# rohitsinghlab/SAME

Hardware: AMD Instinct MI355X
Metric: cell-pairs/sec on 100k×100k cost build + edge-cross sweep; % HBM roofline (higher is better)
Workload: dtype f64

## Files before the change

same_amd/csrc/window_finish.hip:

```cpp
#include "assign.h"
#include "refine.h"

namespace {

using namespace devmath;
using namespace win;
using scan::Pair;

struct FilterArgs {
    const double *xy;
    const int32_t *raw;
    int64_t Tr, n;
    const int32_t *type_id;
    uint8_t *cls;
    double *perim;
    uint8_t *has_kept, *any_valid;
    unsigned long long *best_p;
    unsigned *best_t, *first_v;
    unsigned long long *st_keep, *st_own, *counters;
    int32_t *klist, *nlist, *out;
};

__global__ __launch_bounds__(256) void filter_classify_kernel(Batch<FilterArgs> b, double radius, int angle_enabled, double cos_thr, int near_enabled,
                                                               double tol) {
    const FilterArgs &w = b.w[blockIdx.y];
    if ((int64_t)blockIdx.x * blockDim.x >= w.Tr) return;
    const int64_t t = (int64_t)blockIdx.x * blockDim.x + threadIdx.x;
    const int32_t *__restrict__ tris = w.raw, *__restrict__ type_id = w.type_id;
    bool near = false;
    if (t < w.Tr) {
        const int32_t a = tris[3 * t], bb = tris[3 * t + 1], d = tris[3 * t + 2];
        const TriClass r = classify_triangle(ld2(w.xy, a), ld2(w.xy, bb), ld2(w.xy, d), radius, angle_enabled, cos_thr,
                                             type_id && type_id[a] == type_id[bb] && type_id[bb] == type_id[d]);
        w.cls[t] = r.cls;
        w.perim[t] = r.perim;
        near = near_enabled && r.cls != 1 && fabs(r.maxcos - cos_thr) <= tol;
        if (r.cls == 0 || r.cls == 3) {
            w.any_valid[a] = 1; w.any_valid[bb] = 1; w.any_valid[d] = 1;
            if (r.cls == 0) { w.has_kept[a] = 1; w.has_kept[bb] = 1; w.has_kept[d] = 1; }
        }
        if (w.best_p && r.cls == 3) {
            const unsigned long long key = ~(unsigned long long)__double_as_longlong(r.perim);
            atomicMax(&w.best_p[a], key); atomicMax(&w.best_p[bb], key); atomicMax(&w.best_p[d], key);
        }
    }
    const unsigned long long nb = __ballot(near);
    if ((threadIdx.x & 63) == 0 && nb) atomicAdd(&w.counters[FC_NEAR], (unsigned long long)__builtin_popcountll(nb));
}
__global__ __launch_bounds__(scan::NT) void filter_keep_kernel(Batch<FilterArgs> b) {
    __shared__ scan::Shared sh;
    const FilterArgs &w = b.w[blockIdx.y];
    const int nb = (int)scan::blocks_for(w.Tr);
    if ((int)blockIdx.x >= nb || w.Tr == 0) return;
    const int64_t Tr = w.Tr;
    const uint8_t *__restrict__ cls = w.cls;
    auto val = [&](int64_t t) { return Pair{t < Tr && cls[t] == 0 ? 1u : 0u, 0u}; };
    Pair through;
    const Pair off = scan::exclusive(w.st_keep, (int)blockIdx.x, val, sh, &through);
    const int64_t t = (int64_t)blockIdx.x * scan::NT + threadIdx.x;
    if (t < Tr) {
        const uint8_t c = cls[t];
        if (c == 0) w.klist[off.a] = (int32_t)t;
        if (w.best_p && c == 3) {
            const unsigned long long key = ~(unsigned long long)__double_as_longlong(w.perim[t]);
            for (int q = 0; q < 3; ++q) {
                const int32_t v = w.raw[3 * t + q];
                if (w.best_p[v] == key) atomicMax(&w.best_t[v], ~(unsigned)t);
            }
        }
    }
    if ((int)blockIdx.x == nb - 1 && threadIdx.x == 0) w.counters[FC_KEEP] = through.a;
}
__device__ __forceinline__ bool asks(const uint8_t *has_kept, const uint8_t *any_valid, const unsigned *best_t, int64_t v) {
    return !has_kept[v] && any_valid[v] && best_t[v] != 0u;
}
__global__ __launch_bounds__(256) void filter_first_node_kernel(Batch<FilterArgs> b) {
    const FilterArgs &w = b.w[blockIdx.y];
    const int64_t v = (int64_t)blockIdx.x * blockDim.x + threadIdx.x;
    if (v >= w.n || !asks(w.has_kept, w.any_valid, w.best_t, v)) return;
    atomicMax(&w.first_v[~w.best_t[v]], ~(unsigned)v);
}
__global__ __launch_bounds__(scan::NT) void filter_owner_kernel(Batch<FilterArgs> b) {
    __shared__ scan::Shared sh;
    const FilterArgs &w = b.w[blockIdx.y];
    const int nb = (int)scan::blocks_for(w.n);
    if ((int)blockIdx.x >= nb || w.n == 0) return;
    const int64_t n = w.n;
    auto own = [&](int64_t v) { return v < n && asks(w.has_kept, w.any_valid, w.best_t, v) && w.first_v[~w.best_t[v]] == ~(unsigned)v; };
    auto val = [&](int64_t v) { return Pair{own(v) ? 1u : 0u, 0u}; };
    Pair through;
    const Pair off = scan::exclusive(w.st_own, (int)blockIdx.x, val, sh, &through);
    const int64_t v = (int64_t)blockIdx.x * scan::NT + threadIdx.x;
    if (own(v)) w.nlist[off.a] = (int32_t)v;
    if ((int)blockIdx.x == nb - 1 && threadIdx.x == 0) w.counters[FC_ADD] = through.a;
}
__global__ __launch_bounds__(256) void filter_emit_kernel(Batch<FilterArgs> b) {
    const FilterArgs &w = b.w[blockIdx.y];
    if ((int64_t)blockIdx.x * blockDim.x >= w.Tr) return;
    const int64_t q = (int64_t)blockIdx.x * blockDim.x + threadIdx.x;
    const int64_t n_keep = (int64_t)w.counters[FC_KEEP], n_add = (int64_t)w.counters[FC_ADD];
    if (q == 0) w.counters[FC_TR] = (unsigned long long)(n_keep + n_add);
    if (w.best_p && q < w.Tr && w.cls[q] == 3) {
        bool tie = false;
        for (int c = 0; c < 3; ++c) {
            const int32_t v = w.raw[3 * q + c];
            if (!asks(w.has_kept, w.any_valid, w.best_t, v)) continue;
            const int64_t best = (int64_t)~w.best_t[v];
            tie |= best != q && fabs(w.perim[q] - w.perim[best]) <= 1.8e-15 * w.perim[best];
        }
        if (tie) atomicAdd(&w.counters[FC_TIES], 1ull);
    }
    if (q >= n_keep + n_add) return;
    const int64_t t = q < n_keep ? w.klist[q] : (int64_t)~w.best_t[w.nlist[q - n_keep]];
    w.out[3 * q] = w.raw[3 * t];
    w.out[3 * q + 1] = w.raw[3 * t + 1];
    w.out[3 * q + 2] = w.raw[3 * t + 2];
}


constexpr int WINDOW_GREEDY_ROUNDS = 3;

struct PreferArgs {
    const int32_t *prow;
    const double *cost64, *size_c;
    const unsigned long long *dn;
    uint8_t *alive;
    int32_t *match_pair;
    int64_t cap;
};
__global__ __launch_bounds__(256) void row_prefer_kernel(Batch<PreferArgs> b, double penalty) {
    const PreferArgs &w = b.w[blockIdx.y];
    const int64_t a = (int64_t)blockIdx.x * blockDim.x + threadIdx.x;
    if (a >= w.cap || a >= (int64_t)*w.dn) return;
    const int32_t lo = w.prow[a], hi = w.prow[a + 1];
    double best = __builtin_inf();
    for (int32_t p = lo; p < hi; ++p) {
        const double c = w.cost64[p];
        if (c < best) best = c;
    }
    const uint8_t prefer = best < penalty * w.size_c[a];
    for (int32_t p = lo; p < hi; ++p) w.alive[p] = prefer;
    w.match_pair[a] = -1;
}
struct MatchRowsArgs {
    const int32_t *match_pair, *final_pair, *pairs, *jsec, *prow;
    const uint8_t *alive, *used;
    int64_t n_rows;
    const unsigned long long *dn;
    int32_t *match_loc, *match_row;
    uint8_t *pflag;
    unsigned long long *counters;
};
__global__ __launch_bounds__(256) void match_rows_kernel(Batch<MatchRowsArgs> b) {
    const MatchRowsArgs &w = b.w[blockIdx.y];
    if ((int64_t)blockIdx.x * blockDim.x >= w.n_rows) return;
    const int64_t i = (int64_t)blockIdx.x * blockDim.x + threadIdx.x;
    bool m = false;
    int open = 0;
    if (i < (int64_t)*w.dn) {
        const int32_t p = w.final_pair[i];
        w.match_loc[i] = p >= 0 ? w.pairs[2 * (int64_t)p + 1] : -1;
        w.match_row[i] = p >= 0 ? w.jsec[p] : -1;
        w.pflag[i] = 0;
        m = p >= 0;
        if (w.match_pair[i] < 0 && !w.used[i])
            for (int32_t q = w.prow[i]; q < w.prow[i + 1]; ++q) open += w.alive[q] && !w.used[w.n_rows + w.pairs[2 * (int64_t)q + 1]];
    }
    const unsigned long long bal = __ballot(m), ob = __ballot(open != 0);
    if ((threadIdx.x & 63) == 0) {
        if (bal) atomicAdd(&w.counters[SC_MATCHED], (unsigned long long)__builtin_popcountll(bal));
        if (ob) atomicAdd(&w.counters[SC_REMAINING], (unsigned long long)__builtin_popcountll(ob));
    }
}
__device__ __forceinline__ void cell_flag_or(uint8_t *flags, int32_t i, unsigned bit) {
    atomicOr(reinterpret_cast<unsigned *>(flags) + (i >> 2), bit << (8 * (i & 3)));
}
struct SweepArgs {
    const int32_t *tris;
    int64_t Tr;
    const unsigned long long *dTr;
    const double *axy, *size_c, *ref_xy;
    const int32_t *match_row;
    int8_t *sign;
    double *weight;
    uint8_t *pflag;
    unsigned long long *counters;
};
__global__ __launch_bounds__(256) void window_sweeps_kernel(Batch<SweepArgs> b) {
    const SweepArgs &w = b.w[blockIdx.y];
    if ((int64_t)blockIdx.x * blockDim.x >= w.Tr) return;
    const int32_t *__restrict__ tris = w.tris;
    const double *__restrict__ axy = w.axy, *__restrict__ size_c = w.size_c, *__restrict__ ref_xy = w.ref_xy;
    const int32_t *__restrict__ match_row = w.match_row;
    int8_t *__restrict__ sign = w.sign;
    double *__restrict__ weight = w.weight;
    uint8_t *__restrict__ pflag = w.pflag;
    unsigned long long *__restrict__ counters = w.counters;
    const int64_t t = (int64_t)blockIdx.x * blockDim.x + threadIdx.x;
    const int64_t Tr = w.dTr ? (int64_t)*w.dTr : w.Tr;
    int checked = 0, flipped = 0, ncmp = 0, nviol = 0, tv = 0, aflip = 0, ties = 0;
    if (t < Tr) {
        const int32_t v[3] = {tris[3 * t], tris[3 * t + 1], tris[3 * t + 2]};
        const int32_t m[3] = {match_row[v[0]], match_row[v[1]], match_row[v[2]]};
        double2_t a[3], r[3];
#pragma unroll
        for (int q = 0; q < 3; ++q) {
            a[q] = ld2(axy, v[q]);
            r[q] = m[q] >= 0 ? ld2(ref_xy, m[q]) : double2_t{0.0, 0.0};
        }
        const int8_t ss = orient_sign(a[0], a[1], a[2]);
        sign[t] = ss;
        weight[t] = size_c[v[0]] + size_c[v[1]] + size_c[v[2]];
        const bool all3 = m[0] >= 0 && m[1] >= 0 && m[2] >= 0;
        const uint8_t f = orient_flag(ss, all3, r[0], r[1], r[2]);
        checked = f != 0;
        flipped = f == 2;
        const int E[3][2] = {{0, 1}, {0, 2}, {1, 2}};
#pragma unroll
        for (int e = 0; e < 3; ++e) {
            const int p = E[e][0], q = E[e][1];
            if (m[p] >= 0 && m[q] >= 0) {
                ++ncmp;
                const uint8_t e2 = xyorder_edge(a[p], a[q], r[p], r[q]);
                ties |= a[p].x == a[q].x || a[p].y == a[q].y || r[p].x == r[q].x || r[p].y == r[q].y;
                nviol += ((e2 >> 1) & 1) + ((e2 >> 2) & 1);
                if (e2) { tv = 1; cell_flag_or(pflag, v[p], 1u); cell_flag_or(pflag, v[q], 1u); }
            }
        }
        if (all3) {
            const double bf = signed_area(a[0], a[1], a[2]), af = signed_area(r[0], r[1], r[2]);
            aflip = bf * af < 0.0;
            ties |= sign_in_doubt(a[0], a[1], a[2]) || sign_in_doubt(r[0], r[1], r[2]);
            if (aflip)
                for (int q = 0; q < 3; ++q) cell_flag_or(pflag, v[q], 2u);
        }
    }
    int vals[7] = {checked, flipped, ncmp, nviol, tv, aflip, ties};
#pragma unroll
    for (int q = 0; q < 7; ++q)
#pragma unroll
        for (int off = 32; off > 0; off >>= 1) vals[q] += __shfl_down(vals[q], off, 64);
    __shared__ int part[4][7];
    if ((threadIdx.x & 63) == 0)
        for (int q = 0; q < 7; ++q) part[threadIdx.x >> 6][q] = vals[q];
    __syncthreads();
    if (threadIdx.x < 7) {
        const int s = part[0][threadIdx.x] + part[1][threadIdx.x] + part[2][threadIdx.x] + part[3][threadIdx.x];
        if (s) atomicAdd(&counters[threadIdx.x < 6 ? threadIdx.x : SC_TIES], (unsigned long long)s);
    }
}

struct FilterPlan {
    FilterArgs args{};
    void *zero = nullptr;
    size_t zero_bytes = 0;
    unsigned long long *counters = nullptr;
    bool readd = false;
};

int prepare_filter(same_window *w, const int32_t *d_simplices, int64_t Tr, int ignore_same_type, int ensure_min_triangle_per_node, FilterPlan *plan) {
    same_ctx *ctx = w->ctx;
    const int64_t n = w->n_ua;
    const bool use_type = ignore_same_type && w->has_type;
    plan->readd = use_type && ensure_min_triangle_per_node;
    FilterArgs &a = plan->args;
    a.xy = w->axy_c;
    a.raw = d_simplices;
    a.Tr = Tr;
    a.n = n;
    a.type_id = use_type ? w->type_c : nullptr;
    auto lay = [&](Carver cv) {
        a.st_keep = scan::arg(cv.scan_words(Tr));
        a.st_own = scan::arg(cv.scan_words(n));
        a.counters = plan->counters = cv.take<unsigned long long>(8);
        a.has_kept = cv.take<uint8_t>((size_t)n);
        a.any_valid = cv.take<uint8_t>((size_t)n);
        a.best_p = cv.take<unsigned long long>((size_t)n);
        if (!plan->readd) a.best_p = nullptr;
        a.best_t = cv.take<unsigned>((size_t)n);
        a.first_v = cv.take<unsigned>((size_t)Tr);
        plan->zero_bytes = cv.off;
        a.cls = cv.take<uint8_t>((size_t)Tr);
        a.perim = cv.take<double>((size_t)Tr);
        a.klist = cv.take<int32_t>((size_t)Tr);
        a.nlist = cv.take<int32_t>((size_t)n);
        return cv.off;
    };
    SAME_TRY(ensure(ctx, w->filter, lay(Carver())));
    SAME_TRY(ensure(ctx, w->tris, (size_t)std::max<int64_t>(Tr, 1) * 12));
    lay(Carver(w->filter.p));
    a.out = static_cast<int32_t *>(w->tris.p);
    plan->zero = w->filter.p;
    return SAME_OK;
}

int launch_filter(same_ctx *ctx, FilterPlan *const *plans, int n_w, double radius, int angle_enabled, double cos_thr, double near_tol) {
    Batch<FilterArgs> b{};
    int64_t max_tr = 0, max_n = 0;
    for (int q = 0; q < n_w; ++q) {
        b.w[q] = plans[q]->args;
        max_tr = std::max(max_tr, plans[q]->args.Tr);
        max_n = std::max(max_n, plans[q]->args.n);
    }
    const unsigned nw = (unsigned)n_w;
    const int near_enabled = angle_enabled && cos_thr == cos_thr && cos_thr - cos_thr == 0.0;
    SAME_LAUNCH(ctx, filter_classify_kernel, dim3(grid_for(max_tr), nw), dim3(256), 0, b, radius, angle_enabled, cos_thr, near_enabled, near_tol);
    SAME_LAUNCH(ctx, filter_keep_kernel, dim3(scan::blocks_for(max_tr), nw), dim3(scan::NT), 0, b);
    if (plans[0]->readd) {
        SAME_LAUNCH(ctx, filter_first_node_kernel, dim3(grid_for(max_n), nw), dim3(256), 0, b);
        SAME_LAUNCH(ctx, filter_owner_kernel, dim3(scan::blocks_for(max_n), nw), dim3(scan::NT), 0, b);
    }
    SAME_LAUNCH(ctx, filter_emit_kernel, dim3(grid_for(max_tr), nw), dim3(256), 0, b);
    HIP_TRY(ctx, hipGetLastError());
    return SAME_OK;
}

struct FinishMode {
    int incumbent = SAME_INCUMBENT_GREEDY;
    double no_match_penalty = 0.0;
    int64_t refine_cap = 0;
    double delaunay_penalty = 0.0;
    bool capacity = false;
    same_window_capacity cap{1, 0, 0.0};
    bool has_cap = false;
    int stride = SAME_WINDOW_STATS;
};
int check_mode(same_ctx *ctx, const FinishMode &m) {
    REQUIRE(ctx, m.incumbent == SAME_INCUMBENT_GREEDY || m.incumbent == SAME_INCUMBENT_ASSIGNMENT ||
                     (m.incumbent == SAME_INCUMBENT_TRANSPORT && m.has_cap));
    REQUIRE(ctx, m.refine_cap >= 0 && m.delaunay_penalty >= 0.0 && m.delaunay_penalty - m.delaunay_penalty == 0.0);
    REQUIRE(ctx, m.cap.max_matches >= 1 && m.cap.multiplier >= 0 && m.cap.penalty_coeff >= 0.0 &&
                     m.cap.penalty_coeff - m.cap.penalty_coeff == 0.0);
    return SAME_OK;
}
FinishMode mode_of(int incumbent, double no_match_penalty, int64_t refine_rounds_cap, double delaunay_penalty,
                   const same_window_capacity *capacity, bool wide) {
    FinishMode m{incumbent, no_match_penalty, refine_rounds_cap, delaunay_penalty};
    m.capacity = capacity != nullptr && refine_rounds_cap > 0;
    if (capacity) m.cap = *capacity;
    m.has_cap = capacity != nullptr;
    m.stride = !wide ? SAME_WINDOW_STATS : incumbent == SAME_INCUMBENT_TRANSPORT ? SAME_WINDOW_STATS_TRANSPORT : SAME_WINDOW_STATS_CAP;
    return m;
}
enum { WS_AS_FLAGS = 8, WS_AS_OBJ = 9, WS_REFINE = 10, WS_AS_EXTRA = 16 };

struct FinishPlan : FinishBack {
    FinishMode mode;
    unsigned long long *zero = nullptr;
    void *filter_zero = nullptr;
    size_t filter_zero_bytes = 0;
    same_greedy_state gs;
    int32_t *match_pair = nullptr;
    int64_t cap_tr = 0;
    const unsigned long long *dTr = nullptr;
    asg::AssignArgs aargs{};
    bool refine = false;
    rfn::RefineArgs rargs{};
};

int enqueue_tail(same_ctx *ctx, same_window *const *ws, FinishPlan *const *ps, int n_w) {
    Batch<MatchRowsArgs> mb{};
    Batch<SweepArgs> sb{};
    int64_t max_n = 0, max_tr = 0;
    for (int q = 0; q < n_w; ++q) {
        same_window *w = ws[q];
        FinishPlan *p = ps[q];
        const int64_t n = w->n_ua;
        mb.w[q] = MatchRowsArgs{p->match_pair, p->refine ? p->rargs.match : p->match_pair, w->pairs, w->jsec, w->prow, p->gs.alive, p->gs.used, n, w->counts + 2, w->match_loc, p->match_row, p->pflag,
                                p->counters};
        sb.w[q] = SweepArgs{static_cast<const int32_t *>(w->tris.p), p->cap_tr, p->dTr, w->axy_c, w->size_c, w->ref->xy, p->match_row, w->sign, w->weight,
                            p->pflag, p->counters};
        max_n = std::max(max_n, n);
        max_tr = std::max(max_tr, p->cap_tr);
    }
    if (max_n) SAME_LAUNCH(ctx, match_rows_kernel, dim3(grid_for(max_n), (unsigned)n_w), dim3(256), 0, mb);
    if (max_tr) SAME_LAUNCH(ctx, window_sweeps_kernel, dim3(grid_for(max_tr), (unsigned)n_w), dim3(256), 0, sb);
    HIP_TRY(ctx, hipGetLastError());
    return SAME_OK;
}

int prepare_finish(same_window *w, const int32_t *host_tris, int64_t cap_tr, const unsigned long long *dTr, const FinishMode &mode,
                   FinishPlan *p) {
    same_ctx *ctx = w->ctx;
    const int64_t n = w->n_ua, P = w->P, n_ends = n + w->n_r;
    const size_t tt = (size_t)std::max<int64_t>(cap_tr, 1);
    p->mode = mode;
    p->cap_tr = cap_tr;
    p->dTr = dTr;
    p->gs.float_costs = w->cost_f32 != 0;
    p->aargs = asg::AssignArgs{};
    p->aargs.n = n;
    p->aargs.n_r = w->n_r;
    p->aargs.transport = mode.incumbent == SAME_INCUMBENT_TRANSPORT;
    p->aargs.pc = mode.cap.penalty_coeff;
    p->refine = mode.refine_cap > 0;
    rfn::RefineArgs &r = p->rargs;
    r = rfn::RefineArgs{};
    r.n = n;
    r.n_r = w->n_r;
    r.cap_tr = cap_tr;
    auto lay = [&](Carver cv) {
        p->gs.used = cv.take<uint8_t>((size_t)n_ends);
        p->gs.key[0] = cv.take<unsigned long long>((size_t)n_ends * 2);
        p->gs.idx[0] = cv.take<unsigned>((size_t)n_ends * 2);
        win::lay(*p, cv, n);
        p->gs.sel = p->sel;
        p->gs.alive = cv.take<uint8_t>((size_t)std::max<int64_t>(P, 1));
        p->match_pair = cv.take<int32_t>((size_t)n);
        w->match_loc = cv.take<int32_t>((size_t)n);
        w->sign = cv.take<int8_t>(tt);
        w->weight = cv.take<double>(tt);
        if (mode.incumbent != SAME_INCUMBENT_GREEDY) asg::lay(p->aargs, cv);
        if (p->refine) rfn::lay(r, cv);
        return cv.off;
    };
    SAME_TRY(ensure(ctx, w->finish, lay(Carver())));
    SAME_TRY(ensure(ctx, w->tris, tt * 12));
    lay(Carver(w->finish.p));
    p->zero = static_cast<unsigned long long *>(w->finish.p);
    p->gs.key[1] = p->gs.key[0] + n_ends;
    p->gs.idx[1] = p->gs.idx[0] + n_ends;
    w->match_row = p->match_row;
    w->pflag = p->pflag;
    if (p->refine) {
        r.prow = w->prow;
        r.pairs = w->pairs;
        r.cost = w->cost64;
        r.size = w->size_c;
        r.dp = mode.delaunay_penalty;
        r.axy = w->axy_c;
        r.ref_xy = w->ref->xy;
        r.ref_row = w->jsec;
        r.tris = static_cast<const int32_t *>(w->tris.p);
        r.dTr = dTr;
        r.cap = mode.refine_cap;
        r.penalty = mode.no_match_penalty;
        if (mode.capacity) {
            r.pc = mode.cap.penalty_coeff;
            r.rsize = w->ref->size;
            r.ref_rows = w->rows_r;
            r.P = P;
            r.lim_row = w->lim_row;
            r.lim_P = w->lim_P;
            r.max_matches = mode.cap.max_matches;
            r.multiplier = mode.cap.multiplier;
        }
        r.start = p->match_pair;
        r.ctrl = p->counters + SC_REFINE;
    }
    REQUIRE(ctx, w->host_finish_off + p->back_bytes <= w->host_filter_off);
    if (host_tris && cap_tr) SAME_COPY(ctx, w->tris.p, host_tris, (size_t)cap_tr * 12, hipMemcpyHostToDevice);
    return SAME_OK;
}

int enqueue_refine(same_ctx *ctx, FinishPlan *const *ps, int n_w) {
    rfn::RefineArgs jobs[SAME_LAUNCH_WINDOWS];
    int k = 0;
    for (int q = 0; q < n_w; ++q)
        if (ps[q]->refine) jobs[k++] = ps[q]->rargs;
    if (k == 0) return SAME_OK;
    SAME_TRY(rfn::launch_setup(ctx, jobs, k));
    return rfn::launch_rounds(ctx, jobs, k, rfn::FIRST_ROUNDS);
}

int launch_finish(same_ctx *ctx, same_window *const *ws, FinishPlan *const *ps, int n_w) {
    const double no_match_penalty = ps[0]->mode.no_match_penalty;
    if (ps[0]->mode.incumbent != SAME_INCUMBENT_GREEDY) {
        const bool transport = ps[0]->mode.incumbent == SAME_INCUMBENT_TRANSPORT;
        asg::AssignArgs jobs[SAME_LAUNCH_WINDOWS];
        if (transport) {
            rfn::RefineArgs lim[SAME_LAUNCH_WINDOWS];
            for (int q = 0; q < n_w; ++q) {
                const same_window *w = ws[q];
                const same_window_capacity &c = ps[q]->mode.cap;
                rfn::RefineArgs &r = lim[q];
                r = rfn::RefineArgs{};
                r.rsize = w->ref->size;
                r.ref_row = w->jsec;
                r.ref_rows = w->rows_r;
                r.P = w->P;
                r.lim_row = w->lim_row;
                r.lim_P = w->lim_P;
                r.n_r = w->n_r;
                r.max_matches = c.max_matches;
                r.multiplier = c.multiplier;
                r.limit = ps[q]->aargs.limit;
            }
            SAME_TRY(rfn::launch_limits(ctx, lim, n_w));
        }
        for (int q = 0; q < n_w; ++q) {
            same_window *w = ws[q];
            FinishPlan *p = ps[q];
            asg::AssignArgs &a = jobs[q];
            a = p->aargs;
            a.prow = w->prow;
            a.pairs = w->pairs;
            a.cost = w->cost64;
            a.size = w->size_c;
            a.penalty = no_match_penalty;
            a.max_pops = asg::default_max_pops(w->n_ua, w->n_r, w->P, transport);
            a.alive = p->gs.alive;
            a.match_pair = p->match_pair;
            a.res = p->gs.sel;
        }
        SAME_TRY(asg::launch(ctx, jobs, n_w));
        SAME_TRY(enqueue_refine(ctx, ps, n_w));
        return enqueue_tail(ctx, ws, ps, n_w);
    }
    Batch<PreferArgs> pb{};
    same_greedy_job jobs[SAME_LAUNCH_WINDOWS];
    int64_t max_n = 0;
    for (int q = 0; q < n_w; ++q) {
        same_window *w = ws[q];
        FinishPlan *p = ps[q];
        pb.w[q] = PreferArgs{w->prow, w->cost64, w->size_c, w->counts + 2, p->gs.alive, p->match_pair, w->n_ua};
        jobs[q].pairs = w->pairs;
        jobs[q].costs = w->cost64;
        jobs[q].P = w->P;
        jobs[q].n_m = w->n_ua;
        jobs[q].n_r = w->n_r;
        jobs[q].st = p->gs;
        jobs[q].match_pair = p->match_pair;
        max_n = std::max(max_n, w->n_ua);
    }
    if (max_n) SAME_LAUNCH(ctx, row_prefer_kernel, dim3(grid_for(max_n), (unsigned)n_w), dim3(256), 0, pb, no_match_penalty);
    SAME_TRY(same_greedy_rounds_batch_core(ctx, jobs, n_w, 0, WINDOW_GREEDY_ROUNDS));
    SAME_TRY(enqueue_refine(ctx, ps, n_w));
    return enqueue_tail(ctx, ws, ps, n_w);
}

int enqueue_finish_copy(same_window *w, FinishPlan *p) {
    same_ctx *ctx = w->ctx;
    SAME_COPY(ctx, static_cast<char *>(w->host) + w->host_finish_off, reinterpret_cast<const char *>(p->gs.sel), p->back_bytes, hipMemcpyDeviceToHost);
    return SAME_OK;
}

int settle(same_window *w, FinishPlan *p, bool fresh, int64_t *out_stats) {
    same_ctx *ctx = w->ctx;
    char *h = static_cast<char *>(w->host) + w->host_finish_off;
    const unsigned long long *rc = reinterpret_cast<const unsigned long long *>(h + p->o_counters) + SC_REFINE;
    bool redo = fresh;
    if (p->refine) {
        int chunk = rfn::FIRST_ROUNDS;
        if (fresh) {
            SAME_TRY(enqueue_refine(ctx, &p, 1));
            SAME_COPY(ctx, const_cast<unsigned long long *>(rc), p->rargs.ctrl, rfn::RC_COUNT * 8, hipMemcpyDeviceToHost);
            SAME_WAIT(ctx);
        }
        const int64_t cap = p->mode.refine_cap;
        while (!rc[rfn::RC_SETTLED] && (int64_t)rc[rfn::RC_ROUNDS] < cap) {
            chunk = (int)std::min<int64_t>(std::min(2 * chunk, 256), cap - (int64_t)rc[rfn::RC_ROUNDS]);
            SAME_TRY(rfn::launch_rounds(ctx, &p->rargs, 1, chunk));
            SAME_COPY(ctx, const_cast<unsigned long long *>(rc), p->rargs.ctrl, rfn::RC_COUNT * 8, hipMemcpyDeviceToHost);
            SAME_WAIT(ctx);
            ++ctx->stats[SAME_STAT_GREEDY_READBACKS];
            redo = true;
        }
    }
    if (redo) {
        SAME_FILL(ctx, p->counters, 0, SC_REFINE * 8);
        SAME_TRY(enqueue_tail(ctx, &w, &p, 1));
        SAME_COPY(ctx, h, reinterpret_cast<const char *>(p->gs.sel), p->back_bytes, hipMemcpyDeviceToHost);
        SAME_WAIT(ctx);
    }
    if (p->refine) {
        int64_t *rf = out_stats + WS_REFINE;
        rf[0] = (int64_t)rc[rfn::RC_ROUNDS];
        rf[1] = (int64_t)rc[rfn::RC_MOVES];
        rf[2] = (int64_t)rc[rfn::RC_SETTLED];
        rf[3] = (int64_t)rc[rfn::RC_OBJ0];
        rf[4] = (int64_t)rc[rfn::RC_OBJ];
        if (p->mode.stride > SAME_WINDOW_STATS) rf[5] = (int64_t)rc[rfn::RC_EXTRA];
    }
    return SAME_OK;
}

int read_finish(same_window *w, FinishPlan *p, int32_t *out_match_row, uint8_t *out_point_flag, int64_t *out_stats, int64_t *out_ties) {
    same_ctx *ctx = w->ctx;
    const int64_t n = w->n_ua, P = w->P;
    char *h = static_cast<char *>(w->host) + w->host_finish_off;
    const char *dsel = reinterpret_cast<const char *>(p->gs.sel);
    const unsigned long long *sel = reinterpret_cast<const unsigned long long *>(h);
    const unsigned long long *cnt = reinterpret_cast<const unsigned long long *>(h + p->o_counters);
    int rounds = 0;
    bool again = false;
    if (p->mode.incumbent != SAME_INCUMBENT_GREEDY) {
        rounds = (int)sel[0];
        out_stats[WS_AS_FLAGS] = (int64_t)sel[2];
        out_stats[WS_AS_OBJ] = (int64_t)sel[3];
        if (p->mode.incumbent == SAME_INCUMBENT_TRANSPORT) out_stats[WS_AS_EXTRA] = (int64_t)sel[4];
    } else if (P) {
        int q = 0;
        while (q < WINDOW_GREEDY_ROUNDS && sel[q] != 0) ++q;
        rounds = q;
        if (q == WINDOW_GREEDY_ROUNDS && cnt[SC_REMAINING] != 0) {
            int batch = 4;
            for (;;) {
                REQUIRE(ctx, rounds <= P + 1);
                SAME_FILL(ctx, p->gs.sel, 0, (size_t)batch * 8);
                SAME_TRY(same_greedy_rounds_core(ctx, w->pairs, w->cost64, P, nullptr, n, w->n_r, p->gs, p->match_pair, rounds, batch));
                SAME_COPY(ctx, h, dsel, (size_t)batch * 8, hipMemcpyDeviceToHost);
                SAME_WAIT(ctx);
                ++ctx->stats[SAME_STAT_GREEDY_READBACKS];
                q = 0;
                while (q < batch && sel[q] != 0) ++q;
                rounds += q;
                if (q < batch) break;
                if (batch < SAME_GREEDY_BATCH_MAX) batch *= 2;
            }
            again = true;
        }
    }
    SAME_TRY(settle(w, p, again, out_stats));
    for (int q = 0; q < 8; ++q) out_stats[q] = (int64_t)cnt[q];
    out_stats[SC_ROUNDS] = rounds;
    *out_ties += (int64_t)cnt[SC_TIES];
    memcpy(out_match_row, h + p->o_match_row, (size_t)n * sizeof(int32_t));
    memcpy(out_point_flag, h + p->o_pflag, (size_t)n);
    return SAME_OK;
}

}

static int filter_finish(same_window *const *windows, int n_windows, int source, const int32_t *simplices, const int64_t *simplex_offsets,
                         double radius, int angle_enabled, double cos_thr, double near_tol, int ignore_same_type,
                         int ensure_min_triangle_per_node, const FinishMode &mode, int32_t *out_match_row, uint8_t *out_point_flag,
                         int64_t *out_stats, int64_t *out_counts) {
    same_ctx *ctx = nullptr;
    SAME_TRY(check_batch(windows, n_windows, &ctx));
    SAME_TRY(check_mode(ctx, mode));
    REQUIRE(ctx, source == SAME_TRIS_SIMPLICES || source == SAME_TRIS_KEPT || source == SAME_TRIS_DEVICE || source == SAME_TRIS_CALLER);
    const bool from_caller = source == SAME_TRIS_CALLER;
    const bool on_device = source == SAME_TRIS_DEVICE || from_caller;
    REQUIRE(ctx, on_device == !simplices && on_device == !simplex_offsets);
    std::vector<int64_t> dd_offsets;
    if (on_device) {
        dd_offsets.assign((size_t)n_windows + 1, 0);
        for (int i = 0; i < n_windows; ++i) {
            REQUIRE(ctx, (from_caller ? windows[i]->caller_ok : windows[i]->dd_ok) && windows[i]->staged == 2);
            dd_offsets[(size_t)i + 1] = dd_offsets[(size_t)i] + (from_caller ? windows[i]->n_caller : windows[i]->n_dd);
        }
        simplex_offsets = dd_offsets.data();
    }
    REQUIRE(ctx, out_counts && out_stats && simplex_offsets[0] == 0);
    int64_t n_cells = 0;
    for (int i = 0; i < n_windows; ++i) {
        const int64_t Tr = simplex_offsets[i + 1] - simplex_offsets[i];
        REQUIRE(ctx, windows[i]->staged == 2 && Tr >= 0 && Tr < ((int64_t)1 << 31) - 512);
        n_cells += windows[i]->n_ua;
    }
    REQUIRE(ctx, n_cells == 0 || (out_match_row && out_point_flag));
    for (int q = 0; q < 4 * n_windows; ++q) out_counts[q] = 0;
    for (int q = 0; q < mode.stride * n_windows; ++q) out_stats[q] = 0;
    SAME_TRY(same_use(ctx));
    if (!on_device)
        for (int i = 0; i < n_windows; ++i)
            SAME_TRY(check_index_range(ctx, simplices + 3 * simplex_offsets[i], (simplex_offsets[i + 1] - simplex_offsets[i]) * 3, 0,
                                       windows[i]->n_ua, "triangles"));
    struct Item {
        FilterPlan fplan;
        FinishPlan plan;
        bool filtered = false, enqueued = false;
    };
    std::vector<Item> items((size_t)n_windows);
    const int32_t *d_simplices = nullptr;
    if (source == SAME_TRIS_SIMPLICES && simplex_offsets[n_windows] > 0) {
        int32_t *d = nullptr;
        SAME_TRY(slot_as(ctx, SL_TRIS, (size_t)simplex_offsets[n_windows] * 3, &d));
        SAME_COPY(ctx, d, simplices, (size_t)simplex_offsets[n_windows] * 12, hipMemcpyHostToDevice);
        d_simplices = d;
    }
    int rc = SAME_OK;
    std::vector<same_window *> live;
    std::vector<FinishPlan *> plans;
    std::vector<FilterPlan *> fplans;
    for (int i = 0; i < n_windows && rc == SAME_OK; ++i) {
        same_window *w = windows[i];
        Item &it = items[(size_t)i];
        const int32_t *tri = on_device ? nullptr : simplices + 3 * simplex_offsets[i];
        const int64_t Tr = simplex_offsets[i + 1] - simplex_offsets[i];
        w->filtered = w->finished = 0;
        w->Tr = 0;
        if (w->n_ua == 0) continue;
        if (Tr && source != SAME_TRIS_KEPT) {
            const int32_t *raw = from_caller ? w->caller_out : on_device ? static_cast<const int32_t *>(w->dd_tris.p) : d_simplices + 3 * simplex_offsets[i];
            rc = prepare_filter(w, raw, Tr, ignore_same_type, ensure_min_triangle_per_node, &it.fplan);
            if (rc == SAME_OK) rc = prepare_finish(w, nullptr, Tr, it.fplan.counters + FC_TR, mode, &it.plan);
            if (rc == SAME_OK) {
                fplans.push_back(&it.fplan);
                it.plan.filter_zero = it.fplan.zero;
                it.plan.filter_zero_bytes = it.fplan.zero_bytes;
            }
            it.filtered = true;
        } else {
            rc = prepare_finish(w, Tr ? tri : nullptr, Tr, nullptr, mode, &it.plan);
        }
        if (rc == SAME_OK) {
            live.push_back(w);
            plans.push_back(&it.plan);
        }
    }
    for (size_t g = 0; g < live.size() && rc == SAME_OK; g += SAME_LAUNCH_WINDOWS) {
        ZeroArgs zr[SAME_LAUNCH_WINDOWS];
        const int n_g = (int)std::min<size_t>(SAME_LAUNCH_WINDOWS, live.size() - g);
        for (int q = 0; q < n_g; ++q) {
            const FinishPlan *fp = plans[g + (size_t)q];
            zr[q] = ZeroArgs{{fp->zero, fp->filter_zero}, {fp->zero_bytes, fp->filter_zero_bytes}};
        }
        rc = launch_zero(ctx, zr, n_g);
    }
    for (size_t g = 0, e; g < fplans.size() && rc == SAME_OK; g = e) {
        for (e = g + 1; e < fplans.size() && e - g < SAME_LAUNCH_WINDOWS && fplans[e]->readd == fplans[g]->readd; ++e) {}
        rc = launch_filter(ctx, fplans.data() + g, (int)(e - g), radius, angle_enabled, cos_thr, near_tol);
    }
    for (size_t g = 0, e; g < live.size() && rc == SAME_OK; g = e) {
        for (e = g + 1; e < live.size() && e - g < SAME_LAUNCH_WINDOWS && live[e]->cost_f32 == live[g]->cost_f32; ++e) {}
        rc = launch_finish(ctx, live.data() + g, plans.data() + g, (int)(e - g));
    }
    {
        CopyArgs ca[SAME_LAUNCH_WINDOWS];
        int n_g = 0;
        for (int i = 0; i < n_windows && rc == SAME_OK; ++i) {
            same_window *w = windows[i];
            Item &it = items[(size_t)i];
            if (w->n_ua != 0) {
                if (w->host_dev) {
                    ca[n_g++] = CopyArgs{{it.plan.gs.sel, it.filtered ? it.fplan.counters : nullptr},
                                         {w->host_dev + w->host_finish_off, w->host_dev + w->host_filter_off},
                                         {it.plan.back_bytes, it.filtered ? FC_COPIED * sizeof(unsigned long long) : 0}};
                } else {
                    if (it.filtered) {
                        unsigned long long *hf = reinterpret_cast<unsigned long long *>(static_cast<char *>(w->host) + w->host_filter_off);
                        hipError_t e = hipMemcpyAsync(hf, it.fplan.counters, FC_COPIED * sizeof(unsigned long long), hipMemcpyDeviceToHost, ctx->stream);
                        ++ctx->stats[SAME_STAT_COPIES];
                        if (e != hipSuccess) rc = same_fail(ctx, SAME_EIO, "filter counters", e);
                    }
                    if (rc == SAME_OK) rc = enqueue_finish_copy(w, &it.plan);
                }
                it.enqueued = rc == SAME_OK;
            }
            if (rc == SAME_OK && n_g && (n_g == SAME_LAUNCH_WINDOWS || i == n_windows - 1)) {
                rc = launch_copy_back(ctx, ca, n_g);
                n_g = 0;
            }
        }
    }
    if (rc != SAME_OK) {
        (void)hipStreamSynchronize(ctx->stream);
        return rc;
    }
    SAME_WAIT(ctx);
    int64_t cell0 = 0;
    for (int i = 0; i < n_windows; ++i) {
        same_window *w = windows[i];
        Item &it = items[(size_t)i];
        const int64_t Tr = simplex_offsets[i + 1] - simplex_offsets[i];
        int64_t *counts = out_counts + 4 * i, *stats = out_stats + mode.stride * i;
        if (!it.enqueued) {
            w->filtered = w->finished = 1;
            continue;
        }
        int32_t *const match_out = out_match_row + cell0;
        uint8_t *const flag_out = out_point_flag + cell0;
        cell0 += w->n_ua;
        if (it.filtered) {
            const unsigned long long *hf = reinterpret_cast<const unsigned long long *>(static_cast<const char *>(w->host) + w->host_filter_off);
            const int64_t n_keep = (int64_t)hf[FC_KEEP], n_near = (int64_t)hf[FC_NEAR], n_add = it.fplan.readd ? (int64_t)hf[FC_ADD] : 0;
            counts[0] = n_keep;
            counts[1] = n_add;
            counts[2] = n_near;
            counts[3] = (int64_t)hf[FC_TIES];
            if (n_near) continue;
            w->Tr = n_keep + n_add;
        } else {
            counts[0] = Tr;
            w->Tr = Tr;
        }
        SAME_TRY(read_finish(w, &it.plan, match_out, flag_out, stats, counts + 3));
        w->filtered = w->finished = 1;
    }
    return SAME_OK;
}

static int refinish(same_window *window, const int32_t *match_pair, const FinishMode &mode, int32_t *out_match_row, uint8_t *out_point_flag,
                    int64_t *out_stats) {
    if (!window) return SAME_EINVAL;
    same_window *w = window;
    same_ctx *ctx = w->ctx;
    SAME_TRY(check_mode(ctx, mode));
    REQUIRE(ctx, w->finished && w->staged == 2 && w->n_ua > 0 && match_pair && out_match_row && out_point_flag && out_stats);
    for (int64_t i = 0; i < w->n_ua; ++i) REQUIRE(ctx, match_pair[i] >= -1 && match_pair[i] < w->P);
    SAME_TRY(same_use(ctx));
    FinishPlan p;
    SAME_TRY(prepare_finish(w, nullptr, w->Tr, nullptr, mode, &p));
    SAME_FILL(ctx, p.zero, 0, p.zero_bytes);
    if (w->P) SAME_FILL(ctx, p.gs.alive, 0, (size_t)w->P);
    SAME_COPY(ctx, p.match_pair, match_pair, (size_t)w->n_ua * 4, hipMemcpyHostToDevice);
    FinishPlan *pp = &p;
    SAME_TRY(enqueue_refine(ctx, &pp, 1));
    SAME_TRY(enqueue_tail(ctx, &w, &pp, 1));
    char *h = static_cast<char *>(w->host) + w->host_finish_off;
    SAME_COPY(ctx, h, reinterpret_cast<const char *>(p.gs.sel), p.back_bytes, hipMemcpyDeviceToHost);
    SAME_WAIT(ctx);
    for (int q = 0; q < mode.stride; ++q) out_stats[q] = 0;
    SAME_TRY(settle(w, &p, false, out_stats));
    const unsigned long long *cnt = reinterpret_cast<const unsigned long long *>(h + p.o_counters);
    for (int q = 0; q < 8; ++q) out_stats[q] = (int64_t)cnt[q];
    memcpy(out_match_row, h + p.o_match_row, (size_t)w->n_ua * sizeof(int32_t));
    memcpy(out_point_flag, h + p.o_pflag, (size_t)w->n_ua);
    return SAME_OK;
}

extern "C" {

int same_window_filter_finish(same_window *const *windows, int n_windows, int source, const int32_t *simplices, const int64_t *simplex_offsets,
                              double radius, int angle_enabled, double cos_thr, double near_tol, int ignore_same_type,
                              int ensure_min_triangle_per_node, double no_match_penalty, int incumbent, int64_t refine_rounds_cap,
                              double delaunay_penalty, int32_t *out_match_row, uint8_t *out_point_flag, int64_t *out_stats,
                              int64_t *out_counts) {
    return filter_finish(windows, n_windows, source, simplices, simplex_offsets, radius, angle_enabled, cos_thr, near_tol, ignore_same_type,
                         ensure_min_triangle_per_node, mode_of(incumbent, no_match_penalty, refine_rounds_cap, delaunay_penalty, nullptr, false),
                         out_match_row, out_point_flag, out_stats, out_counts);
}

int same_window_filter_finish_cap(same_window *const *windows, int n_windows, int source, const int32_t *simplices,
                                  const int64_t *simplex_offsets, double radius, int angle_enabled, double cos_thr, double near_tol,
                                  int ignore_same_type, int ensure_min_triangle_per_node, double no_match_penalty, int incumbent,
                                  int64_t refine_rounds_cap, double delaunay_penalty, const same_window_capacity *capacity,
                                  int32_t *out_match_row, uint8_t *out_point_flag, int64_t *out_stats, int64_t *out_counts) {
    return filter_finish(windows, n_windows, source, simplices, simplex_offsets, radius, angle_enabled, cos_thr, near_tol, ignore_same_type,
                         ensure_min_triangle_per_node, mode_of(incumbent, no_match_penalty, refine_rounds_cap, delaunay_penalty, capacity, true),
                         out_match_row, out_point_flag, out_stats, out_counts);
}

int same_window_refinish(same_window *window, const int32_t *match_pair, double no_match_penalty, int64_t refine_rounds_cap,
                         double delaunay_penalty, int32_t *out_match_row, uint8_t *out_point_flag, int64_t *out_stats) {
    return refinish(window, match_pair, mode_of(SAME_INCUMBENT_GREEDY, no_match_penalty, refine_rounds_cap, delaunay_penalty, nullptr, false),
                    out_match_row, out_point_flag, out_stats);
}

int same_window_refinish_cap(same_window *window, const int32_t *match_pair, double no_match_penalty, int64_t refine_rounds_cap,
                             double delaunay_penalty, const same_window_capacity *capacity, int32_t *out_match_row,
                             uint8_t *out_point_flag, int64_t *out_stats) {
    return refinish(window, match_pair, mode_of(SAME_INCUMBENT_GREEDY, no_match_penalty, refine_rounds_cap, delaunay_penalty, capacity, true),
                    out_match_row, out_point_flag, out_stats);
}

}
```

Measured before the change: 609.2 billion.

## Fuse triangle filter classify/keep scan and owner/emit into fewer kernels

Merges triangle classification with the keep-compaction scan so kept triangles are written directly to the output, removing the klist buffer and a kernel launch. The first-node atomic pass and separate emit kernel are replaced by a per-node check against the other vertices of its best triangle, fused with the owner scan and output write. This cuts launches and intermediate buffers (first_v, klist, nlist). The trade-off is that the scan value lambda may recompute the classification for neighbouring indices. The emit kernel now only runs when the re-add path is active, so FC_TR is set in the classify kernel otherwise.

```diff
diff --git a/same_amd/csrc/window_finish.hip b/same_amd/csrc/window_finish.hip
--- a/same_amd/csrc/window_finish.hip
+++ b/same_amd/csrc/window_finish.hip
@@ -16,91 +16,89 @@
     double *perim;
     uint8_t *has_kept, *any_valid;
     unsigned long long *best_p;
-    unsigned *best_t, *first_v;
+    unsigned *best_t;
     unsigned long long *st_keep, *st_own, *counters;
-    int32_t *klist, *nlist, *out;
+    int32_t *out;
 };
 
-__global__ __launch_bounds__(256) void filter_classify_kernel(Batch<FilterArgs> b, double radius, int angle_enabled, double cos_thr, int near_enabled,
-                                                               double tol) {
-    const FilterArgs &w = b.w[blockIdx.y];
-    if ((int64_t)blockIdx.x * blockDim.x >= w.Tr) return;
-    const int64_t t = (int64_t)blockIdx.x * blockDim.x + threadIdx.x;
-    const int32_t *__restrict__ tris = w.raw, *__restrict__ type_id = w.type_id;
-    bool near = false;
-    if (t < w.Tr) {
-        const int32_t a = tris[3 * t], bb = tris[3 * t + 1], d = tris[3 * t + 2];
-        const TriClass r = classify_triangle(ld2(w.xy, a), ld2(w.xy, bb), ld2(w.xy, d), radius, angle_enabled, cos_thr,
-                                             type_id && type_id[a] == type_id[bb] && type_id[bb] == type_id[d]);
-        w.cls[t] = r.cls;
-        w.perim[t] = r.perim;
-        near = near_enabled && r.cls != 1 && fabs(r.maxcos - cos_thr) <= tol;
-        if (r.cls == 0 || r.cls == 3) {
-            w.any_valid[a] = 1; w.any_valid[bb] = 1; w.any_valid[d] = 1;
-            if (r.cls == 0) { w.has_kept[a] = 1; w.has_kept[bb] = 1; w.has_kept[d] = 1; }
-        }
-        if (w.best_p && r.cls == 3) {
-            const unsigned long long key = ~(unsigned long long)__double_as_longlong(r.perim);
-            atomicMax(&w.best_p[a], key); atomicMax(&w.best_p[bb], key); atomicMax(&w.best_p[d], key);
-        }
-    }
-    const unsigned long long nb = __ballot(near);
-    if ((threadIdx.x & 63) == 0 && nb) atomicAdd(&w.counters[FC_NEAR], (unsigned long long)__builtin_popcountll(nb));
-}
-__global__ __launch_bounds__(scan::NT) void filter_keep_kernel(Batch<FilterArgs> b) {
+
+__global__ __launch_bounds__(scan::NT) void filter_classify_keep_kernel(Batch<FilterArgs> b, double radius, int angle_enabled, double cos_thr,
+                                                                        int near_enabled, double tol) {
     __shared__ scan::Shared sh;
     const FilterArgs &w = b.w[blockIdx.y];
     const int nb = (int)scan::blocks_for(w.Tr);
     if ((int)blockIdx.x >= nb || w.Tr == 0) return;
     const int64_t Tr = w.Tr;
-    const uint8_t *__restrict__ cls = w.cls;
-    auto val = [&](int64_t t) { return Pair{t < Tr && cls[t] == 0 ? 1u : 0u, 0u}; };
+    const int64_t t = (int64_t)blockIdx.x * scan::NT + threadIdx.x;
+    const int32_t *__restrict__ tris = w.raw, *__restrict__ type_id = w.type_id;
+    const double *__restrict__ xy = w.xy;
+    auto classify = [&](int64_t i) {
+        const int32_t a = tris[3 * i], bb = tris[3 * i + 1], d = tris[3 * i + 2];
+        return classify_triangle(ld2(xy, a), ld2(xy, bb), ld2(xy, d), radius, angle_enabled, cos_thr,
+                                 type_id && type_id[a] == type_id[bb] && type_id[bb] == type_id[d]);
+    };
+    bool near = false, keep = false;
+    int32_t a = 0, bb = 0, d = 0;
+    if (t < Tr) {
+        a = tris[3 * t]; bb = tris[3 * t + 1]; d = tris[3 * t + 2];
+        const TriClass r = classify(t);
+        w.cls[t] = r.cls;
+        w.perim[t] = r.perim;
+        keep = r.cls == 0;
+        near = near_enabled && r.cls != 1 && fabs(r.maxcos - cos_thr) <= tol;
+        if (r.cls == 0 || r.cls == 3) {
+            w.any_valid[a] = 1; w.any_valid[bb] = 1; w.any_valid[d] = 1;
+            if (r.cls == 0) { w.has_kept[a] = 1; w.has_kept[bb] = 1; w.has_kept[d] = 1; }
+        }
+        if (w.best_p && r.cls == 3) {
+            const unsigned long long key = ~(unsigned long long)__double_as_longlong(r.perim);
+            atomicMax(&w.best_p[a], key); atomicMax(&w.best_p[bb], key); atomicMax(&w.best_p[d], key);
+        }
+    }
+    const unsigned long long nbal = __ballot(near);
+    if ((threadIdx.x & 63) == 0 && nbal) atomicAdd(&w.counters[FC_NEAR], (unsigned long long)__builtin_popcountll(nbal));
+    auto val = [&](int64_t i) { return Pair{(i == t ? keep : i < Tr && classify(i).cls == 0) ? 1u : 0u, 0u}; };
     Pair through;
     const Pair off = scan::exclusive(w.st_keep, (int)blockIdx.x, val, sh, &through);
-    const int64_t t = (int64_t)blockIdx.x * scan::NT + threadIdx.x;
-    if (t < Tr) {
-        const uint8_t c = cls[t];
-        if (c == 0) w.klist[off.a] = (int32_t)t;
-        if (w.best_p && c == 3) {
-            const unsigned long long key = ~(unsigned long long)__double_as_longlong(w.perim[t]);
-            for (int q = 0; q < 3; ++q) {
-                const int32_t v = w.raw[3 * t + q];
-                if (w.best_p[v] == key) atomicMax(&w.best_t[v], ~(unsigned)t);
-            }
-        }
-    }
-    if ((int)blockIdx.x == nb - 1 && threadIdx.x == 0) w.counters[FC_KEEP] = through.a;
+    if (keep) {
+        w.out[3 * (int64_t)off.a] = a;
+        w.out[3 * (int64_t)off.a + 1] = bb;
+        w.out[3 * (int64_t)off.a + 2] = d;
+    }
+    if ((int)blockIdx.x == nb - 1 && threadIdx.x == 0) {
+        w.counters[FC_KEEP] = through.a;
+        if (!w.best_p) w.counters[FC_TR] = through.a;
+    }
+}
+__global__ __launch_bounds__(256) void filter_best_kernel(Batch<FilterArgs> b) {
+    const FilterArgs &w = b.w[blockIdx.y];
+    const int64_t t = (int64_t)blockIdx.x * blockDim.x + threadIdx.x;
+    if (t >= w.Tr || w.cls[t] != 3) return;
+    const unsigned long long key = ~(unsigned long long)__double_as_longlong(w.perim[t]);
+    for (int q = 0; q < 3; ++q) {
+        const int32_t v = w.raw[3 * t + q];
+        if (w.best_p[v] == key) atomicMax(&w.best_t[v], ~(unsigned)t);
+    }
 }
 __device__ __forceinline__ bool asks(const uint8_t *has_kept, const uint8_t *any_valid, const unsigned *best_t, int64_t v) {
     return !has_kept[v] && any_valid[v] && best_t[v] != 0u;
 }
-__global__ __launch_bounds__(256) void filter_first_node_kernel(Batch<FilterArgs> b) {
-    const FilterArgs &w = b.w[blockIdx.y];
-    const int64_t v = (int64_t)blockIdx.x * blockDim.x + threadIdx.x;
-    if (v >= w.n || !asks(w.has_kept, w.any_valid, w.best_t, v)) return;
-    atomicMax(&w.first_v[~w.best_t[v]], ~(unsigned)v);
-}
-__global__ __launch_bounds__(scan::NT) void filter_owner_kernel(Batch<FilterArgs> b) {
+__device__ __forceinline__ bool first_to_ask(const FilterArgs &w, int64_t v) {
+    if (v >= w.n || !asks(w.has_kept, w.any_valid, w.best_t, v)) return false;
+    const unsigned bt = w.best_t[v];
+    const int64_t t = (int64_t)~bt;
+    for (int q = 0; q < 3; ++q) {
+        const int64_t u = w.raw[3 * t + q];
+        if (u < v && asks(w.has_kept, w.any_valid, w.best_t, u) && w.best_t[u] == bt) return false;
+    }
+    return true;
+}
+__global__ __launch_bounds__(scan::NT) void filter_owner_emit_kernel(Batch<FilterArgs> b) {
     __shared__ scan::Shared sh;
     const FilterArgs &w = b.w[blockIdx.y];
-    const int nb = (int)scan::blocks_for(w.n);
-    if ((int)blockIdx.x >= nb || w.n == 0) return;
-    const int64_t n = w.n;
-    auto own = [&](int64_t v) { return v < n && asks(w.has_kept, w.any_valid, w.best_t, v) && w.first_v[~w.best_t[v]] == ~(unsigned)v; };
-    auto val = [&](int64_t v) { return Pair{own(v) ? 1u : 0u, 0u}; };
-    Pair through;
-    const Pair off = scan::exclusive(w.st_own, (int)blockIdx.x, val, sh, &through);
-    const int64_t v = (int64_t)blockIdx.x * scan::NT + threadIdx.x;
-    if (own(v)) w.nlist[off.a] = (int32_t)v;
-    if ((int)blockIdx.x == nb - 1 && threadIdx.x == 0) w.counters[FC_ADD] = through.a;
-}
-__global__ __launch_bounds__(256) void filter_emit_kernel(Batch<FilterArgs> b) {
-    const FilterArgs &w = b.w[blockIdx.y];
-    if ((int64_t)blockIdx.x * blockDim.x >= w.Tr) return;
-    const int64_t q = (int64_t)blockIdx.x * blockDim.x + threadIdx.x;
-    const int64_t n_keep = (int64_t)w.counters[FC_KEEP], n_add = (int64_t)w.counters[FC_ADD];
-    if (q == 0) w.counters[FC_TR] = (unsigned long long)(n_keep + n_add);
-    if (w.best_p && q < w.Tr && w.cls[q] == 3) {
+    if (w.Tr == 0 || w.n == 0) return;
+    const int64_t q = (int64_t)blockIdx.x * scan::NT + threadIdx.x;
+    if (q < w.Tr && w.cls[q] == 3) {
         bool tie = false;
         for (int c = 0; c < 3; ++c) {
             const int32_t v = w.raw[3 * q + c];
@@ -110,11 +108,22 @@
         }
         if (tie) atomicAdd(&w.counters[FC_TIES], 1ull);
     }
-    if (q >= n_keep + n_add) return;
-    const int64_t t = q < n_keep ? w.klist[q] : (int64_t)~w.best_t[w.nlist[q - n_keep]];
-    w.out[3 * q] = w.raw[3 * t];
-    w.out[3 * q + 1] = w.raw[3 * t + 1];
-    w.out[3 * q + 2] = w.raw[3 * t + 2];
+    const int nb = (int)scan::blocks_for(w.n);
+    if ((int)blockIdx.x >= nb) return;
+    auto val = [&](int64_t v) { return Pair{first_to_ask(w, v) ? 1u : 0u, 0u}; };
+    Pair through;
+    const Pair off = scan::exclusive(w.st_own, (int)blockIdx.x, val, sh, &through);
+    const int64_t n_keep = (int64_t)w.counters[FC_KEEP];
+    if (first_to_ask(w, q)) {
+        const int64_t t = (int64_t)~w.best_t[q], at = n_keep + (int64_t)off.a;
+        w.out[3 * at] = w.raw[3 * t];
+        w.out[3 * at + 1] = w.raw[3 * t + 1];
+        w.out[3 * at + 2] = w.raw[3 * t + 2];
+    }
+    if ((int)blockIdx.x == nb - 1 && threadIdx.x == 0) {
+        w.counters[FC_ADD] = through.a;
+        w.counters[FC_TR] = (unsigned long long)(n_keep + (int64_t)through.a);
+    }
 }
 
 
@@ -278,12 +287,9 @@
         a.best_p = cv.take<unsigned long long>((size_t)n);
         if (!plan->readd) a.best_p = nullptr;
         a.best_t = cv.take<unsigned>((size_t)n);
-        a.first_v = cv.take<unsigned>((size_t)Tr);
         plan->zero_bytes = cv.off;
         a.cls = cv.take<uint8_t>((size_t)Tr);
         a.perim = cv.take<double>((size_t)Tr);
-        a.klist = cv.take<int32_t>((size_t)Tr);
-        a.nlist = cv.take<int32_t>((size_t)n);
         return cv.off;
     };
     SAME_TRY(ensure(ctx, w->filter, lay(Carver())));
@@ -304,13 +310,12 @@
     }
     const unsigned nw = (unsigned)n_w;
     const int near_enabled = angle_enabled && cos_thr == cos_thr && cos_thr - cos_thr == 0.0;
-    SAME_LAUNCH(ctx, filter_classify_kernel, dim3(grid_for(max_tr), nw), dim3(256), 0, b, radius, angle_enabled, cos_thr, near_enabled, near_tol);
-    SAME_LAUNCH(ctx, filter_keep_kernel, dim3(scan::blocks_for(max_tr), nw), dim3(scan::NT), 0, b);
+    SAME_LAUNCH(ctx, filter_classify_keep_kernel, dim3(scan::blocks_for(max_tr), nw), dim3(scan::NT), 0, b, radius, angle_enabled, cos_thr, near_enabled,
+                near_tol);
     if (plans[0]->readd) {
-        SAME_LAUNCH(ctx, filter_first_node_kernel, dim3(grid_for(max_n), nw), dim3(256), 0, b);
-        SAME_LAUNCH(ctx, filter_owner_kernel, dim3(scan::blocks_for(max_n), nw), dim3(scan::NT), 0, b);
-    }
-    SAME_LAUNCH(ctx, filter_emit_kernel, dim3(grid_for(max_tr), nw), dim3(256), 0, b);
+        SAME_LAUNCH(ctx, filter_best_kernel, dim3(grid_for(max_tr), nw), dim3(256), 0, b);
+        SAME_LAUNCH(ctx, filter_owner_emit_kernel, dim3(scan::blocks_for(std::max(max_n, max_tr)), nw), dim3(scan::NT), 0, b);
+    }
     HIP_TRY(ctx, hipGetLastError());
     return SAME_OK;
 }
```

Result: no change. 609.6 billion, median of 2 (+0.1%).
